# AutoAILab/FusionDepth

Hardware: AMD Instinct MI355X
Metric: training images/sec (640x192, ResNet-18, 4-beam) (higher is better)
Workload: dtype f32

## Files before the change

fusiondepth_amd/csrc/conv.hip:

```cpp
#include "../../include/fdhip.h"
#include "fd_common.h"
#include "conv_fast.h"
#include "conv_generic.h"
#include "conv_wino.h"
#include "conv_limb.h"
#include <stdio.h>
#include <algorithm>
#include "conv_narrow.h"

extern "C" int fd_axpby(const float* a, const float* b, float* out, long n, float alpha, float beta, void* stream);
extern "C" int fd_act_bwd(const float* y, const float* gy, float* gpre, long n, int act, void* stream);

namespace {

__global__ void k_reduce_slabs(const float* __restrict__ slabs, float* __restrict__ out, long n, int splits, int accumulate) {
    for (long i = (long)blockIdx.x * blockDim.x + threadIdx.x; i < n; i += (long)gridDim.x * blockDim.x) {
        float s = accumulate ? out[i] : 0.f;
        for (int z = 0; z < splits; ++z) s += slabs[(long)z * n + i];
        out[i] = s;
    }
}

__global__ void k_weight_relayout(const float* __restrict__ W, float* __restrict__ Wt, int Co, int Ci, int KH, int KW,
                                  int TA, int TB, int kh0, int dkh, int kw0, int dkw) {
// ... 633 lines not shown
        FD_REQUIRE(gy && w && gx, "fd_conv2d_bwd_data: NULL tensor");
        if (int rc = c1_dgrad_launch(d, gy, w, gx, st)) return rc;
        return add_after();
    }
    FD_REQUIRE(gy && w && gx && wt_base, "fd_conv2d_bwd_data: NULL tensor");
    ConvShape s;
    FD_REQUIRE(conv_out_shape(d, s), "fd_conv2d_bwd_data: empty output");
    FD_REQUIRE((long)d->N * d->Cin * (d->H + 2) * (d->W + 2) < (1L << 29) && (long)d->N * d->Cout * s.Ho * s.Wo < (1L << 29),
               "fd_conv2d_bwd_data: tensor too large for 32-bit byte offsets (2 GiB per tensor)");
    const int KH = d->KH, KW = d->KW;
    const long pad_n = d->pad_mode == 1 ? align4((long)d->N * d->Cin * (d->H + 2) * (d->W + 2)) : 0;
    FD_REQUIRE(ws || (pad_n == 0), "fd_conv2d_bwd_data: workspace required for reflect padding");
    float* gpad = ws;
    float* slabs = ws ? ws + pad_n : nullptr;
    if (!wt_ready && d->stride == 1)
        if (int rc = relayout_launch(r, d, w, wt_base, st)) return rc;

    switch (r.fam) {
    case Fam::LIMB_1X1:
        return limb_gemm_launch(wt_base, gy, gx, nullptr, gx_add, ws, d->Cin, d->Cout, d->N, d->H * d->W, 0, st);
    case Fam::WINO:
        return wino_conv_launch(&r.g, gy, wt_base, nullptr, gx, ws, st, gx_add);
    case Fam::WINO_PADDED: {
        const long planes_in = (long)d->N * d->Cout, bx = ((long)(d->H + 2) * (d->W + 2) + 255) / 256;
        float* gyp = slabs + wino_ws_floats(&r.g);
        hipLaunchKernelGGL(k_zero_border_copy, dim3((unsigned)(bx > 64 ? 64 : bx), (unsigned)(planes_in > 32768 ? 32768 : planes_in)), dim3(256), 0, st,
                           gy, gyp, planes_in, d->H, d->W);
        FD_LAUNCH_CHECK("fd_conv2d_bwd_data(zero border)");
        if (int rc = wino_conv_launch(&r.g, gyp, wt_base, nullptr, gpad, slabs, st, nullptr)) return rc;
        reflect_fold_launch(gpad, gx, d, st);
        FD_LAUNCH_CHECK("fd_conv2d_bwd_data(fold)");
        return add_after();
    }
    default: break;
    }
    const bool fast = r.fam != Fam::GENERIC;

    GemmProblem g = {};
    g.X = gy; g.bias = nullptr; g.act = 0; g.in_norm = 0; g.pad_mode = 0;
    g.M = d->Cin; g.Nb = d->N; g.C = d->Cout; g.Hi = s.Ho; g.Wi = s.Wo;
    auto run = [&](const float* A, int TA, int TB, const float* add) -> int {
        if (fast) {
            FastGemmArgs f = {};
            f.A = A; f.X = gy; f.Y = g.Y; f.bias = nullptr;
            f.M = d->Cin; f.C = d->Cout; f.T = TA * TB; f.TB = TB; f.K = f.T * f.C;
            f.Nb = d->N; f.Hi = s.Ho; f.Wi = s.Wo; f.NY = g.NY; f.NX = g.NX;
            f.sy = g.sy; f.oy = g.oy; f.da = g.da; f.sx = g.sx; f.ox = g.ox; f.db = g.db;
            f.pad_mode = 0;
            f.out_ns = g.out_ns; f.out_cs = g.out_cs; f.out_w = g.out_w;
            f.osy = g.osy; f.ooy = g.ooy; f.osx = g.osx; f.oox = g.oox;
            f.out_total = (long)d->N * g.out_ns; f.slab_stride = f.out_total;
            f.slabs = slabs;
            f.add = add;
            return fast_gemm_launch(f, st);
        }
        g.A = A; g.K = d->Cout * TA * TB;
        if (int rc = dispatch_gemm(TA, TB, g, st)) return rc;
        FD_LAUNCH_CHECK("fd_conv2d_bwd_data(gemm)");
        return 0;
    };

    if (d->stride == 1) {
        g.sy = 1; g.da = 1; g.sx = 1; g.db = 1;
        g.osy = 1; g.ooy = 0; g.osx = 1; g.oox = 0;
        if (r.fam == Fam::RING_WINO || r.fam == Fam::RING_N16 || r.fam == Fam::RING_DIRECT) {
            g.NY = d->H; g.NX = d->W; g.oy = -1; g.ox = -1;
            g.Y = gx; g.out_w = d->W; g.out_cs = (long)d->H * d->W; g.out_ns = g.out_cs * d->Cin;
            if (r.fam == Fam::RING_WINO) {
                if (int rc = wino_conv_launch(&r.g, gy, wt_base + r.job[1].off, nullptr, gx, slabs, st, nullptr)) return rc;
            } else if (r.fam == Fam::RING_N16) {
                if (int rc = n16_launch(d, d->Cin, d->Cout, gy, w, nullptr, gx, 1, 0, 0, st)) return rc;
            } else if (int rc = run(wt_base, KH, KW, nullptr)) return rc;
            const int Hp = d->H, Wp2 = d->W + 2;
            const long ring_plane = 2L * Wp2 + 2L * Hp;
            float* ring = gpad;
            FastGemmArgs f = {};
            FastGemmGroup q = {};
            f.A = wt_base; f.X = gy; f.Y = ring; f.bias = nullptr;
            f.M = d->Cin; f.C = d->Cout; f.T = 9; f.TB = 3; f.K = 9 * d->Cout;
            f.Nb = d->N; f.Hi = s.Ho; f.Wi = s.Wo;
            f.sy = 1; f.da = 1; f.sx = 1; f.db = 1; f.pad_mode = 0;
            f.osy = 1; f.osx = 1; f.ooy = 0; f.oox = 0;
            f.out_total = (long)d->N * d->Cin * ring_plane; f.slab_stride = f.out_total; f.slabs = nullptr; f.add = nullptr;
            q.n = 4; q.own_out = 1;
            const int ny[4] = {1, 1, Hp, Hp}, nx[4] = {Wp2, Wp2, 1, 1};
            const int oy4[4] = {-2, -2 + d->H + 1, -1, -1}, ox4[4] = {-2, -2, -2, -2 + d->W + 1};
            const long yoff[4] = {0, Wp2, 2L * Wp2, 2L * Wp2 + Hp};
            for (int j = 0; j < 4; ++j) {
                q.A[j] = wt_base; q.NY[j] = ny[j]; q.NX[j] = nx[j]; q.oy[j] = oy4[j]; q.ox[j] = ox4[j]; q.ooy[j] = 0; q.oox[j] = 0;
                q.T[j] = 9; q.TB[j] = 3; q.K[j] = 9 * d->Cout;
                q.y_off[j] = yoff[j]; q.out_w[j] = nx[j]; q.out_cs[j] = ring_plane; q.out_ns[j] = ring_plane * d->Cin;
            }
            f.NY = q.NY[0]; f.NX = q.NX[0]; f.oy = q.oy[0]; f.ox = q.ox[0];
            f.out_w = q.out_w[0]; f.out_cs = q.out_cs[0]; f.out_ns = q.out_ns[0];
            if (int rc = fast_gemm_group_launch(f, q, st)) return rc;
            const long planes = (long)d->N * d->Cin;
            const int rows2 = (d->H - 2 != 1) ? 2 : 1, cols2 = (d->W - 2 != 1) ? 2 : 1;
            const long targets = planes * ((long)rows2 * d->W + (long)(d->H - rows2) * cols2);
            hipLaunchKernelGGL(k_reflect_ring_fold, dim3((unsigned)ew_blocks(targets)), dim3(256), 0, st, ring, gx, planes, d->H, d->W);
            FD_LAUNCH_CHECK("fd_conv2d_bwd_data(ring fold)");
            return add_after();
        }
        if (d->pad_mode == 1) {
            g.NY = d->H + 2; g.NX = d->W + 2; g.oy = -(KH - 1); g.ox = -(KW - 1);
            g.Y = gpad; g.out_w = d->W + 2;
            g.out_cs = (long)(d->H + 2) * (d->W + 2); g.out_ns = g.out_cs * d->Cin;
            if (int rc = run(wt_base, KH, KW, nullptr)) return rc;
            reflect_fold_launch(gpad, gx, d, st);
            FD_LAUNCH_CHECK("fd_conv2d_bwd_data(fold)");
            return add_after();
        }
        g.NY = d->H; g.NX = d->W; g.oy = -(KH - 1 - d->pad); g.ox = -(KW - 1 - d->pad);
        g.Y = gx; g.out_w = d->W; g.out_cs = (long)d->H * d->W; g.out_ns = g.out_cs * d->Cin;
        const float* add = fast ? gx_add : nullptr;
        if (int rc = run(wt_base, KH, KW, add)) return rc;
        return add ? 0 : add_after();
    }
    g.out_w = d->W; g.out_cs = (long)d->H * d->W; g.out_ns = g.out_cs * d->Cin; g.Y = gx;
    FD_REQUIRE(!r.need_zero || hipMemsetAsync(gx, 0, sizeof(float) * (size_t)gx_n, st) == hipSuccess, "fd_conv2d_bwd_data: memset failed");
    const float* add = fast && !r.need_zero ? gx_add : nullptr;
    if (fast) {
        FastGemmArgs f = {};
        FastGemmGroup q = {};
        f.X = gy; f.Y = gx; f.bias = nullptr;
        f.M = d->Cin; f.C = d->Cout;
        f.Nb = d->N; f.Hi = s.Ho; f.Wi = s.Wo;
        f.sy = 1; f.da = -1; f.sx = 1; f.db = -1;
        f.pad_mode = 0;
        f.out_ns = g.out_ns; f.out_cs = g.out_cs; f.out_w = g.out_w;
        f.osy = 2; f.osx = 2;
        f.out_total = (long)d->N * g.out_ns; f.slab_stride = f.out_total; f.slabs = nullptr;
        f.add = add;
        for (int i = r.njobs - 1; i >= 0; --i) {
            const Job& c = r.job[i];
            if (!wt_ready)
                if (int rc = relayout_launch(r, d, w, wt_base, st, i, 1)) return rc;
            const int j = q.n++;
            q.A[j] = wt_base + c.off; q.NY[j] = (d->H - c.ph + 1) / 2; q.NX[j] = (d->W - c.pw + 1) / 2;
            q.oy[j] = (c.ph + d->pad - c.kh0) / 2; q.ox[j] = (c.pw + d->pad - c.kw0) / 2;
            q.ooy[j] = c.ph; q.oox[j] = c.pw;
            q.T[j] = c.TA * c.TB; q.TB[j] = c.TB; q.K[j] = c.TA * c.TB * d->Cout;
        }
        if (q.n > 0) {
            f.A = q.A[0]; f.NY = q.NY[0]; f.NX = q.NX[0]; f.T = q.T[0]; f.TB = q.TB[0]; f.K = q.K[0];
            if (r.fam == Fam::LIMB_S2) { if (int rc = limb_conv_group_launch(f, q, st)) return rc; }
            else if (int rc = fast_gemm_group_launch(f, q, st)) return rc;
        }
        return add ? 0 : add_after();
    }
    for (int i = 0; i < r.njobs; ++i) {
        const Job& c = r.job[i];
        if (!wt_ready)
            if (int rc = relayout_launch(r, d, w, wt_base, st, i, 1)) return rc;
        g.NY = (d->H - c.ph + 1) / 2; g.NX = (d->W - c.pw + 1) / 2;
        g.sy = 1; g.oy = (c.ph + d->pad - c.kh0) / 2; g.da = -1;
        g.sx = 1; g.ox = (c.pw + d->pad - c.kw0) / 2; g.db = -1;
        g.osy = 2; g.ooy = c.ph; g.osx = 2; g.oox = c.pw;
        if (int rc = run(wt_base + c.off, c.TA, c.TB, nullptr)) return rc;
    }
    return add_after();
}
}

extern "C" long fd_conv2d_fwd_wt_floats(const fd_conv_desc* d) { return d ? route_fwd(d).wt : 0; }
extern "C" long fd_conv2d_fwd_ws_floats(const fd_conv_desc* d) { return d ? route_fwd(d).ws : 0; }

extern "C" int fd_conv2d_fwd(const fd_conv_desc* d, const float* x, const float* w, const float* bias, float* y, float* wt,
                             int wt_ready, float* ws, void* stream) {
    if (int rc = check_desc(d, "fd_conv2d_fwd")) return rc;
    return conv2d_fwd_impl(d, route_fwd(d), x, w, bias, y, wt, wt_ready, ws, nullptr, (hipStream_t)stream);
}
extern "C" int fd_conv2d_fwd_bn_ok(const fd_conv_desc* d, int groups) {
    if (!d || check_desc(d, "fd_conv2d_fwd_bn_ok")) return 0;
    return route_fwd(d).bn && bn_small_slabs_ok(d->N, d->Cout, d->H, d->W, groups) ? 1 : 0;
}
extern "C" int fd_conv2d_fwd_bn(const fd_conv_desc* d, const float* x, const float* w, float* y, float* wt, int wt_ready, float* ws,
                                const float* bn_weight, const float* bn_bias, const float* residual, float* out, float* running_mean,
// ... 151 lines not shown
```

fusiondepth_amd/csrc/conv_fast.h:

```cpp
#pragma once
#include <hip/hip_runtime.h>
#include "../../include/fdhip.h"

struct FastGemmArgs {
    const float* A;
    const float* X;
    float* Y;
    const float* bias;
    float* slabs;
    long slab_stride, out_total;
    int M, K;
    int Nb, C, Hi, Wi;
    int NY, NX;
    int T, TB;
    int sy, oy, da, sx, ox, db;
    int pad_mode;
    long out_ns, out_cs;
    int out_w, osy, ooy, osx, oox;
    int act;
    int xcd_swizzle;
    const float* add;
};

struct FastGemmGroup {
    const float* A[4];
    int NY[4], NX[4], oy[4], ox[4], ooy[4], oox[4], T[4], TB[4], K[4];
    long y_off[4], out_ns[4], out_cs[4];
    int out_w[4];
    int own_out;
    int first_bx[5];
    int n;
};

struct FastWgradArgs {
    const float* dY; const float* X; float* slabs;
    int M, C, T, TB;
    int Nb, Hi, Wi, NY, NX;
    int sy, oy, da, sx, ox, db;
    int pad_mode;
    long dy_ns, dy_cs;
    long pix_per_split;
};

long fast_splitk_slab_floats(const FastGemmArgs& a, int* splits_out);
int fast_gemm_launch(const FastGemmArgs& a, hipStream_t st);
int fast_gemm_group_launch(const FastGemmArgs& a, const FastGemmGroup& q, hipStream_t st);
int fast_weight_relayout(const float* W, float* A2, int Co, int Ci, int KH, int KW, int TA, int TB, int kh0, int dkh, int kw0,
                         int dkw, int mode, hipStream_t st);
int fast_wgrad_splits(int M, int C, int T, long Np);
int fast_wgrad_launch(const FastWgradArgs& a, float* gw, int splits, int accumulate, hipStream_t st);

int fast_splitk_finish_launch(const float* slabs, float* Y, const float* bias, long total, long slab_stride, int splits, long out_cs,
                              int M, int act, hipStream_t st, const float* add = nullptr);

bool n16_shape_ok(const fd_conv_desc* d, int M, int C);
int n16_launch(const fd_conv_desc* d, int M, int C, const float* x, const float* w, const float* bias, float* y, int flip,
               int pad_mode, int act, hipStream_t st);
bool c1_shape_ok(const fd_conv_desc* d);
int c1_fwd_launch(const fd_conv_desc* d, const float* x, const float* w, const float* bias, float* y, hipStream_t st);
int c1_dgrad_launch(const fd_conv_desc* d, const float* gy, const float* w, float* gx, hipStream_t st, const float* x_in = nullptr, int in_act = 0);
bool stem7_fwd_ok(const fd_conv_desc* d);
int stem7_fwd_launch(const fd_conv_desc* d, const float* x, const float* w, const float* bias, float* y, hipStream_t st);
int fast_wgrad_finish_launch(const float* slabs, float* gw, int M, int C, int T, int splits, int accumulate, hipStream_t st);

bool limb_fwd_ok(const fd_conv_desc* d);
bool limb_dgrad_ok(const fd_conv_desc* d);
bool limb_wgrad_ok(const fd_conv_desc* d);
long limb_wt_floats(long M, long K);
long limb_gemm_ws_floats(int M, int K, int Nb, int HW);
int limb_weight_split_launch(const float* w, float* wt, int M, int K, int transposed, hipStream_t st);
int limb_gemm_launch(const float* wt, const float* x, float* y, const float* bias, const float* add, float* ws, int M, int K, int Nb, int HW,
                     int act, hipStream_t st);
long limb_wgrad_ws_floats(int M, int C, int Nb, int HW);
int limb_wgrad_launch(const float* x, const float* gy, float* gw, float* ws, int M, int C, int Nb, int HW, int accumulate, hipStream_t st);
bool limb_conv_problem_ok(int M, int C, int pad_mode, int act);
int limb_conv_weight_split_launch(const float* w, float* wt, int Co, int Ci, int KH, int KW, int TA, int TB, int kh0, int dkh, int kw0, int dkw,
                                  int mode, hipStream_t st);
long limb_conv_ws_floats(const FastGemmArgs& a);
int limb_conv_launch(const FastGemmArgs& a, hipStream_t st);
int limb_conv_group_launch(const FastGemmArgs& a, const FastGemmGroup& q, hipStream_t st);
bool limb_wgrad_s2_shape_ok(int M, int C, int Hi, int Wi, int NY, int NX);
long limb_wgrad_s2_ws_floats(int M, int C, int Nb, int plane, int ntaps);
int limb_wgrad_s2_launch(const float* x, const float* gy, float* gw, float* ws, int M, int C, int Nb, int Hi, int Wi, int NY, int NX, int ntaps,
                         int accumulate, hipStream_t st);
bool limb_conv_1x1_worth(int M, long Np);
```

fusiondepth_amd/csrc/conv_fast.hip:

```cpp
#include "../../include/fdhip.h"
#include "fd_common.h"
#include "conv_fast.h"
#include <type_traits>
#include <stdlib.h>
#include <stdio.h>

#ifndef FD_LS_DIV
#define FD_LS_DIV 2
#endif
namespace {

typedef float f32x16 __attribute__((ext_vector_type(16)));

__device__ __attribute__((noinline)) float act_apply_slow(float v, int act) {
    if (act == 2) return v > 0.f ? v : expm1f(v);
    if (act == 3) return 1.0f / (1.0f + expf(-v));
    return tanhf(v);
}
__device__ __forceinline__ float act_apply(float v, int act) {
    if (act >= 2) return act_apply_slow(v, act);
    return act == 1 ? (v > 0.f ? v : 0.f) : v;
}
__device__ __forceinline__ int refl_idx(int i, int n) {
    i = i < 0 ? -i : i;
    return i >= n ? 2 * n - 2 - i : i;
}

template <int WAVES_M, int WAVES_N, int WM, int WN, int BKC>
__device__ __forceinline__ void conv_fast_body(const FastGemmArgs& g, int bx, int ntx) {
    constexpr int NT = 64 * WAVES_M * WAVES_N;
    constexpr int BM = WAVES_M * 32 * WM, BN = WAVES_N * 32 * WN;
    constexpr int LDA = BM + 1, LDB = BN;
    constexpr int RP = NT / BN;
    constexpr int NB_LOAD = BKC / RP;
    constexpr int A_V4_PER_ROW = BKC / 4;
    constexpr int A_ROWS_PER_PASS = NT / A_V4_PER_ROW;
    constexpr int NA_LOAD = (BM + A_ROWS_PER_PASS - 1) / A_ROWS_PER_PASS;
    constexpr bool A_PARTIAL = (BM % A_ROWS_PER_PASS) != 0;
    static_assert(NT % BN == 0 && BKC % RP == 0, "tile/loader mismatch");
    extern __shared__ __attribute__((aligned(16))) float smem[];
    float* sA = smem;
    float* sB = smem + 2 * BKC * LDA;

    const int tid = threadIdx.x, lane = tid & 63, wave = tid >> 6;
    const int wave_m = wave / WAVES_N, wave_n = wave % WAVES_N;
    if (g.xcd_swizzle) { const int per = ntx >> 3; bx = (bx & 7) * per + (bx >> 3); }
    const int m0 = blockIdx.y * BM;
    const long p0 = (long)bx * BN;
    const int plane = g.NY * g.NX;
    const long Np = (long)g.Nb * plane;
    const unsigned chw = (unsigned)(g.Hi * g.Wi);
    const int cpt = g.C / BKC;
    const int nchunk_all = g.T * cpt;
    const int nsplit = (int)gridDim.z, zs = (int)blockIdx.z;
    const int per_split = (nchunk_all + nsplit - 1) / nsplit;
    const int ch_lo = zs * per_split;
    const int ch_hi = ch_lo + per_split < nchunk_all ? ch_lo + per_split : nchunk_all;

    const int jn = tid % BN;
    const int kr = __builtin_amdgcn_readfirstlane(tid / BN);
    const long pg = p0 + jn;
    const bool pvalid = pg < Np;
    int ry0, cx0;
    unsigned nbase;
    {
        const long pp = pvalid ? pg : 0;
        const int n = (int)(pp / plane);
        const int rem = (int)(pp - (long)n * plane);
        const int y = rem / g.NX, x = rem - y * g.NX;
        ry0 = y * g.sy + g.oy; cx0 = x * g.sx + g.ox;
        nbase = (unsigned)n * (unsigned)g.C * chw;
    }
    const int a4 = tid % A_V4_PER_ROW, ar = tid / A_V4_PER_ROW;

    const __amdgpu_buffer_rsrc_t rsA = fd_make_rsrc(g.A), rsX = fd_make_rsrc(g.X);
    float4 ra[NA_LOAD];
    float rb[NB_LOAD];
    unsigned a_off[NA_LOAD], b_off = FD_OOB;
    const unsigned b_step = 4u * (unsigned)RP * chw;
    int pc_ta, pc_tb, pc_c0;
    { const int t = ch_lo / cpt; pc_c0 = (ch_lo - t * cpt) * BKC; pc_ta = t / g.TB; pc_tb = t - pc_ta * g.TB; }
    const bool refl = g.pad_mode == 1;
    auto prep_chunk = [&](bool live) __attribute__((always_inline)) {
        const unsigned k0 = (unsigned)(pc_ta * g.TB + pc_tb) * (unsigned)g.C + (unsigned)pc_c0;
#pragma unroll
        for (int i = 0; i < NA_LOAD; ++i) {
            int m = m0 + ar + A_ROWS_PER_PASS * i;
            m = m < g.M ? m : g.M - 1;
            a_off[i] = live ? 4u * ((unsigned)m * (unsigned)g.K + k0 + 4u * a4) : FD_OOB;
        }
        int r = ry0 + pc_ta * g.da, cc = cx0 + pc_tb * g.db;
        const bool inb = ((unsigned)r < (unsigned)g.Hi) & ((unsigned)cc < (unsigned)g.Wi);
        const int rr = refl_idx(r, g.Hi), rc = refl_idx(cc, g.Wi);
        r = refl ? rr : r; cc = refl ? rc : cc;
        const bool ok = pvalid & live & (refl | inb);
        b_off = ok ? 4u * (nbase + (unsigned)(pc_c0 + kr) * chw + (unsigned)(r * g.Wi + cc)) : FD_OOB;
        pc_c0 += BKC;
        if (pc_c0 >= g.C) { pc_c0 = 0; ++pc_tb; if (pc_tb >= g.TB) { pc_tb = 0; ++pc_ta; } }
    };
    auto load_a = [&](int i) __attribute__((always_inline)) {
        if (!A_PARTIAL || ar + A_ROWS_PER_PASS * i < BM) ra[i] = fd_ldg128(rsA, a_off[i]);
    };
    auto load_b = [&](int i) __attribute__((always_inline)) { rb[i] = fd_ldg32(rsX, b_off + (unsigned)i * b_step); };
    auto store_a = [&](int buf, int i) __attribute__((always_inline)) {
        if (A_PARTIAL && ar + A_ROWS_PER_PASS * i >= BM) return;
        float* q = sA + buf * BKC * LDA + (4 * a4) * LDA + ar + A_ROWS_PER_PASS * i;
        q[0] = ra[i].x; q[LDA] = ra[i].y; q[2 * LDA] = ra[i].z; q[3 * LDA] = ra[i].w;
    };
    auto store_b = [&](int buf, int i) __attribute__((always_inline)) {
        sB[buf * BKC * LDB + (kr + RP * i) * LDB + jn] = rb[i];
    };

    f32x16 acc[WM][WN];
#pragma unroll
    for (int i = 0; i < WM; ++i)
#pragma unroll
        for (int j = 0; j < WN; ++j)
#pragma unroll
            for (int r = 0; r < 16; ++r) acc[i][j][r] = 0.f;

    constexpr int NK = BKC / 2;
    constexpr int LS = NK / FD_LS_DIV;
    const int arow = lane >> 5, acol = lane & 31;
    if (ch_lo < ch_hi) {
        prep_chunk(true);
#pragma unroll
        for (int i = 0; i < NA_LOAD; ++i) load_a(i);
#pragma unroll
        for (int i = 0; i < NB_LOAD; ++i) load_b(i);
#pragma unroll
        for (int i = 0; i < NA_LOAD; ++i) store_a(0, i);
#pragma unroll
        for (int i = 0; i < NB_LOAD; ++i) store_b(0, i);
        __syncthreads();
        for (int ch = ch_lo; ch < ch_hi; ++ch) {
            const int cur = (ch - ch_lo) & 1;
            prep_chunk(ch + 1 < ch_hi);
            const float* pa = sA + cur * BKC * LDA + arow * LDA + wave_m * 32 * WM + acol;
            const float* pb = sB + cur * BKC * LDB + arow * LDB + wave_n * 32 * WN + acol;
            float av[2][WM], bv[2][WN];
#pragma unroll
            for (int i = 0; i < WM; ++i) av[0][i] = pa[i * 32];
#pragma unroll
            for (int j = 0; j < WN; ++j) bv[0][j] = pb[j * 32];
#pragma unroll
            for (int kk = 0; kk < NK; ++kk) {
                const int cb = kk & 1, nb = cb ^ 1;
                if (kk + 1 < NK) {
#pragma unroll
                    for (int i = 0; i < WM; ++i) av[nb][i] = pa[(kk + 1) * 2 * LDA + i * 32];
#pragma unroll
                    for (int j = 0; j < WN; ++j) bv[nb][j] = pb[(kk + 1) * 2 * LDB + j * 32];
                }
                if (kk < LS) {
#pragma unroll
                    for (int i = 0; i < NA_LOAD; ++i) if ((i * LS) / NA_LOAD == kk) load_a(i);
#pragma unroll
                    for (int i = 0; i < NB_LOAD; ++i) if ((i * LS) / NB_LOAD == kk) load_b(i);
                } else if (kk >= NK - LS) {
#pragma unroll
                    for (int i = 0; i < NA_LOAD; ++i) if ((i * LS) / NA_LOAD == kk - (NK - LS)) store_a(cur ^ 1, i);
#pragma unroll
                    for (int i = 0; i < NB_LOAD; ++i) if ((i * LS) / NB_LOAD == kk - (NK - LS)) store_b(cur ^ 1, i);
                }
                __builtin_amdgcn_sched_barrier(0);
#pragma unroll
                for (int i = 0; i < WM; ++i)
#pragma unroll
                    for (int j = 0; j < WN; ++j)
                        acc[i][j] = __builtin_amdgcn_mfma_f32_32x32x2f32(av[cb][i], bv[cb][j], acc[i][j], 0, 0, 0);
                __builtin_amdgcn_sched_barrier(0);
            }
            __syncthreads();
        }
    }

    const bool final_pass = nsplit == 1;
    const __amdgpu_buffer_rsrc_t rsY = fd_make_rsrc(final_pass ? g.Y : g.slabs + (size_t)blockIdx.z * g.slab_stride);
    const __amdgpu_buffer_rsrc_t rsAdd = fd_make_rsrc(g.add ? g.add : g.Y);
    const bool has_add = final_pass && g.add;
    const unsigned cs4 = 4u * (unsigned)g.out_cs;
    float bias_r[WM][16];
#pragma unroll
    for (int i = 0; i < WM; ++i)
#pragma unroll
        for (int r = 0; r < 16; ++r) bias_r[i][r] = 0.f;
    if (final_pass && g.bias) {
#pragma unroll
        for (int i = 0; i < WM; ++i)
#pragma unroll
            for (int r = 0; r < 16; ++r) {
                const int m = m0 + wave_m * 32 * WM + i * 32 + (r & 3) + 8 * (r >> 2) + 4 * arow;
                bias_r[i][r] = g.bias[m < g.M ? m : g.M - 1];
            }
    }
    auto rows = [&](auto act_tag) __attribute__((always_inline)) {
        constexpr int ACT = decltype(act_tag)::value;
#pragma unroll
        for (int j = 0; j < WN; ++j) {
            const long p = p0 + wave_n * 32 * WN + j * 32 + acol;
            unsigned pix = FD_OOB;
            if (p < Np) {
                const int n = (int)(p / plane);
                const int rem = (int)(p - (long)n * plane);
                const int y = rem / g.NX, x = rem - y * g.NX;
                pix = 4u * (unsigned)((long)n * g.out_ns + (long)(y * g.osy + g.ooy) * g.out_w + (x * g.osx + g.oox));
            }
            unsigned off[WM][16];
            float addv[WM][16];
#pragma unroll
            for (int i = 0; i < WM; ++i)
#pragma unroll
                for (int r = 0; r < 16; ++r) {
                    const int m = m0 + wave_m * 32 * WM + i * 32 + (r & 3) + 8 * (r >> 2) + 4 * arow;
                    off[i][r] = (m < g.M) ? pix + (unsigned)m * cs4 : FD_OOB;
                    addv[i][r] = 0.f;
                }
            if (has_add) {
#pragma unroll
                for (int i = 0; i < WM; ++i)
#pragma unroll
                    for (int r = 0; r < 16; ++r) addv[i][r] = fd_ldg32(rsAdd, off[i][r]);
            }
#pragma unroll
            for (int i = 0; i < WM; ++i)
#pragma unroll
                for (int r = 0; r < 16; ++r) {
                    float v = acc[i][j][r];
                    if (final_pass) {
                        v += bias_r[i][r];
                        if (ACT != 0) v = act_apply(v, g.act);
                        v += addv[i][r];
                    }
                    __builtin_amdgcn_raw_buffer_store_b32(__builtin_bit_cast(unsigned, v), rsY, (int)off[i][r], 0, 0);
                }
        }
    };
    if (g.act == 0 || !final_pass) rows(std::integral_constant<int, 0>{});
    else rows(std::integral_constant<int, -1>{});
}

template <int WAVES_M, int WAVES_N, int WM, int WN, int BKC>
__global__ void __launch_bounds__(64 * WAVES_M * WAVES_N) k_conv_fast(FastGemmArgs g) {
    conv_fast_body<WAVES_M, WAVES_N, WM, WN, BKC>(g, (int)blockIdx.x, (int)gridDim.x);
}

template <int WAVES_M, int WAVES_N, int WM, int WN, int BKC>
__global__ void __launch_bounds__(64 * WAVES_M * WAVES_N) k_conv_fast_grp(FastGemmArgs g, FastGemmGroup q) {
    int j = 0;
    while (j + 1 < q.n && (int)blockIdx.x >= q.first_bx[j + 1]) ++j;
    g.A = q.A[j]; g.NY = q.NY[j]; g.NX = q.NX[j]; g.oy = q.oy[j]; g.ox = q.ox[j]; g.ooy = q.ooy[j]; g.oox = q.oox[j];
    g.T = q.T[j]; g.TB = q.TB[j]; g.K = q.K[j];
    if (q.own_out) { g.Y += q.y_off[j]; g.out_ns = q.out_ns[j]; g.out_cs = q.out_cs[j]; g.out_w = q.out_w[j]; }
    g.xcd_swizzle = 0;
    conv_fast_body<WAVES_M, WAVES_N, WM, WN, BKC>(g, (int)blockIdx.x - q.first_bx[j], q.first_bx[j + 1] - q.first_bx[j]);
}

__global__ void __launch_bounds__(256) k_splitk_finish(const float* __restrict__ slabs, float* __restrict__ Y,
                                                       const float* __restrict__ bias, long total, long slab_stride,
                                                       int splits, long out_cs, int M, int act, const float* __restrict__ add) {
    const unsigned cs = (unsigned)out_cs, uM = (unsigned)M;
    for (unsigned i = blockIdx.x * 256u + threadIdx.x; i < (unsigned)total; i += gridDim.x * 256u) {
        float s = 0.f;
        int z = 0;
        for (; z + 4 <= splits; z += 4) {
            const float a0 = slabs[(size_t)z * slab_stride + i], a1 = slabs[(size_t)(z + 1) * slab_stride + i];
            const float a2 = slabs[(size_t)(z + 2) * slab_stride + i], a3 = slabs[(size_t)(z + 3) * slab_stride + i];
            s += a0; s += a1; s += a2; s += a3;
        }
        for (; z < splits; ++z) s += slabs[(size_t)z * slab_stride + i];
        if (bias) s += bias[(i / cs) % uM];
        s = act_apply(s, act);
        if (add) s += add[i];
        Y[i] = s;
    }
}

template <int WAVES_M, int WAVES_N, int WM, int WN>
__global__ void __launch_bounds__(64 * WAVES_M * WAVES_N) k_wgrad_fast(FastWgradArgs g) {
    constexpr int NT = 64 * WAVES_M * WAVES_N;
    constexpr int BM = WAVES_M * 32 * WM, BN = WAVES_N * 32 * WN;
    constexpr int BP = 32;
    constexpr int LDA = BM + 1, LDB = BN + 1;
    constexpr int RPW = NT / BP;
    constexpr int NA_LOAD = BM / RPW, NB_LOAD = BN / RPW;
    extern __shared__ __attribute__((aligned(16))) float smem[];
    float* sA = smem;
    float* sB = smem + 2 * BP * LDA;

    const int tid = threadIdx.x, lane = tid & 63, wave = tid >> 6;
    const int wave_m = wave / WAVES_N, wave_n = wave % WAVES_N;
    const int cblocks = (g.C + BN - 1) / BN;
    const int t = blockIdx.x / cblocks, c0 = (blockIdx.x - t * cblocks) * BN;
    const int ta = t / g.TB, tb = t - ta * g.TB;
    const int m0 = blockIdx.y * BM;
    const int plane = g.NY * g.NX;
    const long Np = (long)g.Nb * plane;
    const unsigned chw = (unsigned)(g.Hi * g.Wi);
    const long pbeg = (long)blockIdx.z * g.pix_per_split;
    long pend = pbeg + g.pix_per_split;
    if (pend > Np) pend = Np;

    const int pl = tid % BP, rw = tid / BP;
    const int ncol = g.C - c0 < BN ? g.C - c0 : BN;
    const int nrow = g.M - m0 < BM ? g.M - m0 : BM;

    const __amdgpu_buffer_rsrc_t rsY = fd_make_rsrc(g.dY), rsX = fd_make_rsrc(g.X);
    float ra[NA_LOAD], rb[NB_LOAD];
    unsigned rowa[NA_LOAD], rowb[NB_LOAD];
#pragma unroll
    for (int i = 0; i < NA_LOAD; ++i) {
        const int r = rw + RPW * i < nrow ? rw + RPW * i : nrow - 1;
        rowa[i] = 4u * (unsigned)(m0 + r) * (unsigned)g.dy_cs;
    }
#pragma unroll
    for (int i = 0; i < NB_LOAD; ++i) {
        const int c = rw + RPW * i < ncol ? rw + RPW * i : ncol - 1;
        rowb[i] = 4u * (unsigned)(c0 + c) * chw;
    }
    unsigned offa = FD_OOB, offb = FD_OOB;
    int pn, prem;
    { const long p = pbeg + pl; pn = (int)(p / plane); prem = (int)(p - (long)pn * plane); }
    long pcur = pbeg + pl;
    const float inv_nx = 1.0f / (float)g.NX;
    const bool refl = g.pad_mode == 1;
    auto prep_chunk = [&]() __attribute__((always_inline)) {
        const bool pv = pcur < pend;
        int y = (int)(((float)prem + 0.5f) * inv_nx);
        int x = prem - y * g.NX;
        if (x < 0) { --y; x += g.NX; }
        if (x >= g.NX) { ++y; x -= g.NX; }
        offa = pv ? 4u * ((unsigned)pn * (unsigned)g.dy_ns + (unsigned)prem) : FD_OOB;
        int r = y * g.sy + g.oy + ta * g.da, cc = x * g.sx + g.ox + tb * g.db;
        const bool inb = ((unsigned)r < (unsigned)g.Hi) & ((unsigned)cc < (unsigned)g.Wi);
        const int rr = refl_idx(r, g.Hi), rc = refl_idx(cc, g.Wi);
        r = refl ? rr : r; cc = refl ? rc : cc;
        const bool ok = pv & (refl | inb);
        offb = ok ? 4u * ((unsigned)pn * (unsigned)g.C * chw + (unsigned)(r * g.Wi + cc)) : FD_OOB;
// ... 157 lines not shown
                const float h = 0.5f * (t1 + t2);
                v = ky == 0 ? t0 + h : (ky == 1 ? 0.5f * (t1 - t2) : h - t3);
            }
            o[i * os] = old[i] + v;
        }
    }
}

__global__ void __launch_bounds__(256) k_weight_relayout_tc(const float* __restrict__ W, float* __restrict__ A2, int Co,
                                                            int Ci, int KH, int KW, int TA, int TB, int kh0, int dkh, int kw0,
                                                            int dkw, int mode) {
    const int Mr = mode ? Ci : Co, Cr = mode ? Co : Ci;
    const long n = (long)Mr * TA * TB * Cr;
    for (long i = (long)blockIdx.x * 256 + threadIdx.x; i < n; i += (long)gridDim.x * 256) {
        const int c = (int)(i % Cr);
        const int b = (int)((i / Cr) % TB);
        const int a = (int)((i / ((long)Cr * TB)) % TA);
        const int m = (int)(i / ((long)Cr * TB * TA));
        const int co = mode ? c : m, ci = mode ? m : c;
        A2[i] = W[(((long)co * Ci + ci) * KH + kh0 + dkh * a) * KW + kw0 + dkw * b];
    }
}

inline int ew_blocks(long n) {
    long b = (n + 255) / 256;
    return (int)(b < 1 ? 1 : (b > 4096 ? 4096 : b));
}

template <int WAVES_M, int WAVES_N, int WM, int WN, int BKC>
void launch_cfg(const FastGemmArgs& a, int splits, hipStream_t st) {
    constexpr int BM = WAVES_M * 32 * WM, BN = WAVES_N * 32 * WN;
    const long Np = (long)a.Nb * a.NY * a.NX;
    const int gx = fd_cdiv(Np, BN), gy = fd_cdiv(a.M, BM);
    FastGemmArgs g = a;
    g.xcd_swizzle = (gx % 8 == 0 && gx >= 16) ? 1 : 0;
    const size_t lds = sizeof(float) * 2 * BKC * ((BM + 1) + BN);
    fd_launch_lds<k_conv_fast<WAVES_M, WAVES_N, WM, WN, BKC>>(dim3(gx, gy, splits), dim3(64 * WAVES_M * WAVES_N), lds, st, g);
}

}

namespace {
struct FastChoice { int cfg; int splits; };
FastChoice choose_config(const FastGemmArgs& a) {
    if (fd_tun().force_cfg >= 0) {
        const int c = fd_tun().force_cfg, sp = fd_tun().force_splits;
        const bool ok_c = (c == 0 && a.M > 64) || (c == 1 && a.M > 32) || c == 2;
        const bool can = a.osy == 1 && a.osx == 1 && a.slab_stride > 0;
        if (ok_c) return {c, can ? sp : 1};
    }
    const long Np = (long)a.Nb * a.NY * a.NX;
    const int bkc = (a.C % 32 == 0) ? 32 : 16;
    const int nchunk = a.T * (a.C / bkc);
    const bool can_split = a.osy == 1 && a.osx == 1 && a.slab_stride > 0;
    const int bm[3] = {128, 64, 32}, bn[3] = {128, 128, 256};
    const int c = a.M > 32 ? 1 : 2;
    const long tiles = (long)fd_cdiv(Np, bn[c]) * fd_cdiv(a.M, bm[c]);
    const long fill = fd_tun().conv_target;
    int sp = 1;
    if (can_split && tiles < fill) {
        sp = (int)(fill / tiles);
        const int cap = nchunk / 4 > 0 ? (nchunk / 4 < 16 ? nchunk / 4 : 16) : 1;
        if (sp > cap) sp = cap;
        if (sp < 1) sp = 1;
    }
    return {c, sp};
}
}

long fast_splitk_slab_floats(const FastGemmArgs& a, int* splits_out) {
    FastGemmArgs probe = a;
    if (probe.slab_stride <= 0) probe.slab_stride = probe.out_total > 0 ? probe.out_total : 1;
    const FastChoice ch = choose_config(probe);
    if (splits_out) *splits_out = ch.splits;
    return ch.splits > 1 ? (long)ch.splits * a.out_total : 0;
}

namespace {
template <int WAVES_M, int WAVES_N, int WM, int WN, int BKC>
void launch_grp(const FastGemmArgs& a, const FastGemmGroup& q, hipStream_t st) {
    constexpr int BM = WAVES_M * 32 * WM, BN = WAVES_N * 32 * WN;
    FastGemmGroup grp = q;
    int gx = 0;
    for (int j = 0; j < q.n; ++j) { grp.first_bx[j] = gx; gx += fd_cdiv((long)a.Nb * q.NY[j] * q.NX[j], BN); }
    grp.first_bx[q.n] = gx;
    const size_t lds = sizeof(float) * 2 * BKC * ((BM + 1) + BN);
    fd_launch_lds<k_conv_fast_grp<WAVES_M, WAVES_N, WM, WN, BKC>>(dim3(gx, fd_cdiv(a.M, BM), 1), dim3(64 * WAVES_M * WAVES_N), lds, st, a, grp);
}
}

int fast_gemm_group_launch(const FastGemmArgs& a, const FastGemmGroup& q, hipStream_t st) {
    if ((double)a.Nb * a.C * a.Hi * a.Wi * 4.0 >= 2147483648.0) { fd_set_error("conv: tensor exceeds the 2 GiB addressing range of the fast path"); return -1; }
    for (int j = 0; j < q.n; ++j)
        if ((double)a.M * q.K[j] * 4.0 >= 2147483648.0) { fd_set_error("conv: weights exceed the 2 GiB addressing range of the fast path"); return -1; }
    const bool b32 = a.C % 32 == 0;
    long wgs128 = 0;
    for (int j = 0; j < q.n; ++j) wgs128 += fd_cdiv((long)a.Nb * q.NY[j] * q.NX[j], 128) * fd_cdiv(a.M, 64);
    if (a.M > 32 && b32 && wgs128 < (long)fd_tun().grp_tile64_below) launch_grp<2, 2, 1, 1, 32>(a, q, st);
    else if (a.M > 32) { if (b32) launch_grp<2, 2, 1, 2, 32>(a, q, st); else launch_grp<2, 2, 1, 2, 16>(a, q, st); }
    else { if (b32) launch_grp<1, 4, 1, 2, 32>(a, q, st); else launch_grp<1, 4, 1, 2, 16>(a, q, st); }
    hipError_t e = hipGetLastError();
    if (e != hipSuccess) { fd_set_error("k_conv_fast_grp launch failed: %s", hipGetErrorString(e)); return (int)e; }
    return 0;
}

int fast_gemm_launch(const FastGemmArgs& a, hipStream_t st) {
    if ((double)a.Nb * a.C * a.Hi * a.Wi * 4.0 >= 2147483648.0 || (double)a.M * a.K * 4.0 >= 2147483648.0) {
        fd_set_error("conv: tensor exceeds the 2 GiB addressing range of the fast path"); return -1;
    }
    const FastChoice ch = choose_config(a);
    const int splits = ch.splits;
    if (splits > 1 && !a.slabs) { fd_set_error("conv: split-K workspace missing"); return -1; }
    const bool b32 = a.C % 32 == 0;
    if (ch.cfg == 0) {
        if (b32) launch_cfg<2, 2, 2, 2, 32>(a, splits, st); else launch_cfg<2, 2, 2, 2, 16>(a, splits, st);
    } else if (ch.cfg == 1) {
        if (b32) launch_cfg<2, 2, 1, 2, 32>(a, splits, st); else launch_cfg<2, 2, 1, 2, 16>(a, splits, st);
    } else {
        if (b32) launch_cfg<1, 4, 1, 2, 32>(a, splits, st); else launch_cfg<1, 4, 1, 2, 16>(a, splits, st);
    }
    hipError_t e = hipGetLastError();
    if (e != hipSuccess) { fd_set_error("k_conv_fast launch failed: %s", hipGetErrorString(e)); return (int)e; }
    if (splits > 1)
        return fast_splitk_finish_launch(a.slabs, a.Y, a.bias, a.out_total, a.slab_stride, splits, a.out_cs, a.M, a.act, st, a.add);
    return 0;
}

int fast_wgrad_finish_launch(const float* slabs, float* gw, int M, int C, int T, int splits, int accumulate, hipStream_t st) {
    if ((T == 9 && C % 32 == 0) || T == 12) {
        const int cb = (C + 31) / 32;
        int mb = (int)(((long)M * cb) / 1024);
        mb = mb < 1 ? 1 : (mb > 8 ? 8 : mb);
        const dim3 grid(cb, (M + mb - 1) / mb);
#define FD_FIN9(CH, ZU)                                                                                                    \
    do {                                                                                                                   \
        if (T == 9) hipLaunchKernelGGL((k_wgrad_finish9<9, CH, ZU>), grid, dim3(384), 0, st, slabs, gw, M, C, splits, accumulate, mb); \
        else hipLaunchKernelGGL((k_wgrad_finish9<12, CH, ZU>), grid, dim3(384), 0, st, slabs, gw, M, C, splits, accumulate, mb);       \
    } while (0)
        static_assert(FIN9_MB == 8, "the mb rule above and the CH choice below end at 8 channels");
        if (mb == 1) FD_FIN9(1, 16);
        else if (mb == 2) FD_FIN9(2, 8);
        else if (mb <= 4) FD_FIN9(4, 4);
        else if (splits > 1) FD_FIN9(8, 2);
        else FD_FIN9(8, 1);
#undef FD_FIN9
        hipError_t e9 = hipGetLastError();
        if (e9 != hipSuccess) { fd_set_error("k_wgrad_finish9 launch failed: %s", hipGetErrorString(e9)); return (int)e9; }
        return 0;
    }
    hipLaunchKernelGGL(k_wgrad_finish, dim3(ew_blocks((long)M * C * T)), dim3(256), 0, st, slabs, gw, M, C, T, splits, accumulate);
    hipError_t e = hipGetLastError();
    if (e != hipSuccess) { fd_set_error("k_wgrad_finish launch failed: %s", hipGetErrorString(e)); return (int)e; }
    return 0;
}

int fast_splitk_finish_launch(const float* slabs, float* Y, const float* bias, long total, long slab_stride, int splits, long out_cs,
                              int M, int act, hipStream_t st, const float* add) {
    hipLaunchKernelGGL(k_splitk_finish, dim3(ew_blocks(total)), dim3(256), 0, st, slabs, Y, bias, total, slab_stride, splits, out_cs, M,
                       act, add);
    hipError_t e = hipGetLastError();
    if (e != hipSuccess) { fd_set_error("k_splitk_finish launch failed: %s", hipGetErrorString(e)); return (int)e; }
    return 0;
}

int fast_weight_relayout(const float* W, float* A2, int Co, int Ci, int KH, int KW, int TA, int TB, int kh0, int dkh,
                         int kw0, int dkw, int mode, hipStream_t st) {
    const long n = (long)Co * Ci * TA * TB;
    hipLaunchKernelGGL(k_weight_relayout_tc, dim3(ew_blocks(n)), dim3(256), 0, st, W, A2, Co, Ci, KH, KW, TA, TB, kh0, dkh,
                       kw0, dkw, mode);
    hipError_t e = hipGetLastError();
    if (e != hipSuccess) { fd_set_error("k_weight_relayout_tc launch failed: %s", hipGetErrorString(e)); return (int)e; }
    return 0;
}

int fast_wgrad_splits(int M, int C, int T, long Np) {
    const long target = fd_tun().wgrad_target;
    const int bn = C >= 128 ? 128 : 64;
    const long tiles = (long)T * fd_cdiv(C, bn) * fd_cdiv(M, M > 32 ? 64 : 32);
    long sp = target / tiles;
    const long maxs = (Np + 511) / 512;
    if (sp > maxs) sp = maxs;
// ... 27 lines not shown
```

Measured before the change: 705.7.

## Restrict ring dgrad taps to live window and fold reflection in epilogue

The reflect-pad ring correction in the dgrad path now computes only the kernel taps that actually reach each border strip (a tap window given by ta0/tb0/TBW) instead of all nine. A new ring epilogue accumulates directly into gx, with a fifth group covering the corners, so the separate ring buffer and the reflect-fold kernel are skipped. The small-tile threshold is also raised for these thin groups. This removes redundant MACs, one kernel launch and a round trip through the intermediate buffer. In exchange it adds read-modify-write stores, shuffle-based corner reductions and more complex indexing, which risks correctness bugs and races at overlapping outputs.

```diff
diff --git a/fusiondepth_amd/csrc/conv.hip b/fusiondepth_amd/csrc/conv.hip
--- a/fusiondepth_amd/csrc/conv.hip
+++ b/fusiondepth_amd/csrc/conv.hip
@@ -739,17 +739,31 @@
             f.sy = 1; f.da = 1; f.sx = 1; f.db = 1; f.pad_mode = 0;
             f.osy = 1; f.osx = 1; f.ooy = 0; f.oox = 0;
             f.out_total = (long)d->N * d->Cin * ring_plane; f.slab_stride = f.out_total; f.slabs = nullptr; f.add = nullptr;
-            q.n = 4; q.own_out = 1;
+            q.n = 4; q.own_out = 1; q.thin = 1;
             const int ny[4] = {1, 1, Hp, Hp}, nx[4] = {Wp2, Wp2, 1, 1};
             const int oy4[4] = {-2, -2 + d->H + 1, -1, -1}, ox4[4] = {-2, -2, -2, -2 + d->W + 1};
             const long yoff[4] = {0, Wp2, 2L * Wp2, 2L * Wp2 + Hp};
+            const int ta0[4] = {2, 0, 0, 0}, tb0[4] = {0, 0, 2, 0}, tbn[4] = {3, 3, 1, 1};
             for (int j = 0; j < 4; ++j) {
                 q.A[j] = wt_base; q.NY[j] = ny[j]; q.NX[j] = nx[j]; q.oy[j] = oy4[j]; q.ox[j] = ox4[j]; q.ooy[j] = 0; q.oox[j] = 0;
-                q.T[j] = 9; q.TB[j] = 3; q.K[j] = 9 * d->Cout;
+                q.T[j] = 3; q.TB[j] = tbn[j]; q.K[j] = 9 * d->Cout;
+                q.ta0[j] = ta0[j]; q.tb0[j] = tb0[j]; q.TBW[j] = 3;
                 q.y_off[j] = yoff[j]; q.out_w[j] = nx[j]; q.out_cs[j] = ring_plane; q.out_ns[j] = ring_plane * d->Cin;
             }
             f.NY = q.NY[0]; f.NX = q.NX[0]; f.oy = q.oy[0]; f.ox = q.ox[0];
             f.out_w = q.out_w[0]; f.out_cs = q.out_cs[0]; f.out_ns = q.out_ns[0];
+            if (d->H >= 4 && d->W >= 4) {
+                q.own_out = 0;
+                for (int j = 0; j < 4; ++j) q.ring_kind[j] = j;
+                q.A[4] = wt_base; q.NY[4] = 4; q.NX[4] = 4; q.oy[4] = 0; q.ox[4] = 0; q.ooy[4] = 0; q.oox[4] = 0;
+                q.T[4] = 9; q.TB[4] = 3; q.K[4] = 9 * d->Cout; q.ta0[4] = 0; q.tb0[4] = 0; q.TBW[4] = 3; q.ring_kind[4] = 4;
+                q.n = 5;
+                f.Y = gx; f.ring_h = d->H; f.ring_w = d->W;
+                f.out_w = d->W; f.out_cs = (long)d->H * d->W; f.out_ns = f.out_cs * d->Cin;
+                f.out_total = (long)d->N * f.out_ns; f.slab_stride = f.out_total;
+                if (int rc = fast_gemm_group_launch(f, q, st)) return rc;
+                return add_after();
+            }
             if (int rc = fast_gemm_group_launch(f, q, st)) return rc;
             const long planes = (long)d->N * d->Cin;
             const int rows2 = (d->H - 2 != 1) ? 2 : 1, cols2 = (d->W - 2 != 1) ? 2 : 1;
diff --git a/fusiondepth_amd/csrc/conv_fast.h b/fusiondepth_amd/csrc/conv_fast.h
--- a/fusiondepth_amd/csrc/conv_fast.h
+++ b/fusiondepth_amd/csrc/conv_fast.h
@@ -20,15 +20,23 @@
     int act;
     int xcd_swizzle;
     const float* add;
+    int ta0, tb0, TBW;
+    int ring_h, ring_w;
+    int ring_kind;
 };
 
+constexpr int FAST_GRP_MAX = 5;
 struct FastGemmGroup {
-    const float* A[4];
-    int NY[4], NX[4], oy[4], ox[4], ooy[4], oox[4], T[4], TB[4], K[4];
-    long y_off[4], out_ns[4], out_cs[4];
-    int out_w[4];
+    const float* A[FAST_GRP_MAX];
+    int NY[FAST_GRP_MAX], NX[FAST_GRP_MAX], oy[FAST_GRP_MAX], ox[FAST_GRP_MAX], ooy[FAST_GRP_MAX], oox[FAST_GRP_MAX];
+    int T[FAST_GRP_MAX], TB[FAST_GRP_MAX], K[FAST_GRP_MAX];
+    int ta0[FAST_GRP_MAX], tb0[FAST_GRP_MAX], TBW[FAST_GRP_MAX];
+    int ring_kind[FAST_GRP_MAX];
+    long y_off[FAST_GRP_MAX], out_ns[FAST_GRP_MAX], out_cs[FAST_GRP_MAX];
+    int out_w[FAST_GRP_MAX];
     int own_out;
-    int first_bx[5];
+    int thin;
+    int first_bx[FAST_GRP_MAX + 1];
     int n;
 };
 
diff --git a/fusiondepth_amd/csrc/conv_fast.hip b/fusiondepth_amd/csrc/conv_fast.hip
--- a/fusiondepth_amd/csrc/conv_fast.hip
+++ b/fusiondepth_amd/csrc/conv_fast.hip
@@ -1,6 +1,7 @@
 #include "../../include/fdhip.h"
 #include "fd_common.h"
 #include "conv_fast.h"
+#include <algorithm>
 #include <type_traits>
 #include <stdlib.h>
 #include <stdio.h>
@@ -26,7 +27,8 @@
     return i >= n ? 2 * n - 2 - i : i;
 }
 
-template <int WAVES_M, int WAVES_N, int WM, int WN, int BKC>
+constexpr int EPI_STORE = 0, EPI_RING = 1;
+template <int WAVES_M, int WAVES_N, int WM, int WN, int BKC, bool WIN = false, int EPI = EPI_STORE>
 __device__ __forceinline__ void conv_fast_body(const FastGemmArgs& g, int bx, int ntx) {
     constexpr int NT = 64 * WAVES_M * WAVES_N;
     constexpr int BM = WAVES_M * 32 * WM, BN = WAVES_N * 32 * WN;
@@ -60,7 +62,7 @@
     const int jn = tid % BN;
     const int kr = __builtin_amdgcn_readfirstlane(tid / BN);
     const long pg = p0 + jn;
-    const bool pvalid = pg < Np;
+    bool pvalid = pg < Np;
     int ry0, cx0;
     unsigned nbase;
     {
@@ -70,6 +72,12 @@
         const int y = rem / g.NX, x = rem - y * g.NX;
         ry0 = y * g.sy + g.oy; cx0 = x * g.sx + g.ox;
         nbase = (unsigned)n * (unsigned)g.C * chw;
+        if (EPI == EPI_RING && g.ring_kind == 4) {
+            const int py = x == 2 ? ((y >> 1) ? g.ring_h - 1 : 2) : ((y >> 1) ? g.ring_h + 1 : 0);
+            const int px = x == 0 ? ((y & 1) ? g.ring_w - 1 : 2) : ((y & 1) ? g.ring_w + 1 : 0);
+            ry0 = py - 2; cx0 = px - 2;
+            pvalid = pvalid && x < 3;
+        }
     }
     const int a4 = tid % A_V4_PER_ROW, ar = tid / A_V4_PER_ROW;
 
@@ -79,10 +87,12 @@
     unsigned a_off[NA_LOAD], b_off = FD_OOB;
     const unsigned b_step = 4u * (unsigned)RP * chw;
     int pc_ta, pc_tb, pc_c0;
-    { const int t = ch_lo / cpt; pc_c0 = (ch_lo - t * cpt) * BKC; pc_ta = t / g.TB; pc_tb = t - pc_ta * g.TB; }
+    const int tb_lo = WIN ? g.tb0 : 0, tb_hi = tb_lo + g.TB, tbw = WIN ? g.TBW : g.TB;
+    { const int t = ch_lo / cpt; pc_c0 = (ch_lo - t * cpt) * BKC; pc_ta = t / g.TB; pc_tb = t - pc_ta * g.TB + tb_lo; }
+    if (WIN) pc_ta += g.ta0;
     const bool refl = g.pad_mode == 1;
     auto prep_chunk = [&](bool live) __attribute__((always_inline)) {
-        const unsigned k0 = (unsigned)(pc_ta * g.TB + pc_tb) * (unsigned)g.C + (unsigned)pc_c0;
+        const unsigned k0 = (unsigned)(pc_ta * tbw + pc_tb) * (unsigned)g.C + (unsigned)pc_c0;
 #pragma unroll
         for (int i = 0; i < NA_LOAD; ++i) {
             int m = m0 + ar + A_ROWS_PER_PASS * i;
@@ -96,7 +106,7 @@
         const bool ok = pvalid & live & (refl | inb);
         b_off = ok ? 4u * (nbase + (unsigned)(pc_c0 + kr) * chw + (unsigned)(r * g.Wi + cc)) : FD_OOB;
         pc_c0 += BKC;
-        if (pc_c0 >= g.C) { pc_c0 = 0; ++pc_tb; if (pc_tb >= g.TB) { pc_tb = 0; ++pc_ta; } }
+        if (pc_c0 >= g.C) { pc_c0 = 0; ++pc_tb; if (pc_tb >= tb_hi) { pc_tb = tb_lo; ++pc_ta; } }
     };
     auto load_a = [&](int i) __attribute__((always_inline)) {
         if (!A_PARTIAL || ar + A_ROWS_PER_PASS * i < BM) ra[i] = fd_ldg128(rsA, a_off[i]);
@@ -236,6 +246,45 @@
                 }
         }
     };
+    if constexpr (EPI == EPI_RING) {
+        const int H = g.ring_h, W = g.ring_w, kind = g.ring_kind;
+#pragma unroll
+        for (int j = 0; j < WN; ++j) {
+            const long p = p0 + wave_n * 32 * WN + j * 32 + acol;
+            unsigned pix = FD_OOB;
+            if (p < Np) {
+                const int n = (int)(p / plane);
+                const int rem = (int)(p - (long)n * plane);
+                const int y = rem / g.NX, x = rem - y * g.NX;
+                int ty, tx;
+                bool on;
+                if (kind <= 1) { on = !(x == 0 || x == 2 || x == W - 1 || x == W + 1); ty = kind ? H - 2 : 1; tx = x - 1; }
+                else if (kind <= 3) { on = !(y == 1 || y == H - 2); ty = y; tx = kind == 3 ? W - 2 : 1; }
+                else { on = x == 0; ty = (y >> 1) ? H - 2 : 1; tx = (y & 1) ? W - 2 : 1; }
+                if (on) pix = 4u * (unsigned)((long)n * g.out_ns + (long)ty * W + tx);
+            }
+            unsigned off[WM][16];
+            float old[WM][16];
+#pragma unroll
+            for (int i = 0; i < WM; ++i)
+#pragma unroll
+                for (int r = 0; r < 16; ++r) {
+                    const int m = m0 + wave_m * 32 * WM + i * 32 + (r & 3) + 8 * (r >> 2) + 4 * arow;
+                    off[i][r] = (m < g.M) ? pix + (unsigned)m * cs4 : FD_OOB;
+                    old[i][r] = fd_ldg32(rsY, off[i][r]);
+                }
+#pragma unroll
+            for (int i = 0; i < WM; ++i)
+#pragma unroll
+                for (int r = 0; r < 16; ++r) {
+                    const float v = acc[i][j][r];
+                    float s = 0.f + v;
+                    if (kind == 4) { s += __shfl_down(v, 1); s += __shfl_down(v, 2); }
+                    __builtin_amdgcn_raw_buffer_store_b32(__builtin_bit_cast(unsigned, old[i][r] + s), rsY, (int)off[i][r], 0, 0);
+                }
+        }
+        return;
+    }
     if (g.act == 0 || !final_pass) rows(std::integral_constant<int, 0>{});
     else rows(std::integral_constant<int, -1>{});
 }
@@ -245,15 +294,16 @@
     conv_fast_body<WAVES_M, WAVES_N, WM, WN, BKC>(g, (int)blockIdx.x, (int)gridDim.x);
 }
 
-template <int WAVES_M, int WAVES_N, int WM, int WN, int BKC>
+template <int WAVES_M, int WAVES_N, int WM, int WN, int BKC, int EPI>
 __global__ void __launch_bounds__(64 * WAVES_M * WAVES_N) k_conv_fast_grp(FastGemmArgs g, FastGemmGroup q) {
     int j = 0;
     while (j + 1 < q.n && (int)blockIdx.x >= q.first_bx[j + 1]) ++j;
     g.A = q.A[j]; g.NY = q.NY[j]; g.NX = q.NX[j]; g.oy = q.oy[j]; g.ox = q.ox[j]; g.ooy = q.ooy[j]; g.oox = q.oox[j];
     g.T = q.T[j]; g.TB = q.TB[j]; g.K = q.K[j];
+    g.ta0 = q.ta0[j]; g.tb0 = q.tb0[j]; g.TBW = q.TBW[j]; g.ring_kind = q.ring_kind[j];
     if (q.own_out) { g.Y += q.y_off[j]; g.out_ns = q.out_ns[j]; g.out_cs = q.out_cs[j]; g.out_w = q.out_w[j]; }
     g.xcd_swizzle = 0;
-    conv_fast_body<WAVES_M, WAVES_N, WM, WN, BKC>(g, (int)blockIdx.x - q.first_bx[j], q.first_bx[j + 1] - q.first_bx[j]);
+    conv_fast_body<WAVES_M, WAVES_N, WM, WN, BKC, true, EPI>(g, (int)blockIdx.x - q.first_bx[j], q.first_bx[j + 1] - q.first_bx[j]);
 }
 
 __global__ void __launch_bounds__(256) k_splitk_finish(const float* __restrict__ slabs, float* __restrict__ Y,
@@ -577,10 +627,15 @@
     constexpr int BM = WAVES_M * 32 * WM, BN = WAVES_N * 32 * WN;
     FastGemmGroup grp = q;
     int gx = 0;
-    for (int j = 0; j < q.n; ++j) { grp.first_bx[j] = gx; gx += fd_cdiv((long)a.Nb * q.NY[j] * q.NX[j], BN); }
+    for (int j = 0; j < q.n; ++j) {
+        grp.first_bx[j] = gx; gx += fd_cdiv((long)a.Nb * q.NY[j] * q.NX[j], BN);
+        if (grp.TBW[j] == 0) { grp.TBW[j] = q.TB[j]; grp.ta0[j] = 0; grp.tb0[j] = 0; }
+    }
     grp.first_bx[q.n] = gx;
     const size_t lds = sizeof(float) * 2 * BKC * ((BM + 1) + BN);
-    fd_launch_lds<k_conv_fast_grp<WAVES_M, WAVES_N, WM, WN, BKC>>(dim3(gx, fd_cdiv(a.M, BM), 1), dim3(64 * WAVES_M * WAVES_N), lds, st, a, grp);
+    const dim3 grid(gx, fd_cdiv(a.M, BM), 1), block(64 * WAVES_M * WAVES_N);
+    if (a.ring_h) fd_launch_lds<k_conv_fast_grp<WAVES_M, WAVES_N, WM, WN, BKC, EPI_RING>>(grid, block, lds, st, a, grp);
+    else fd_launch_lds<k_conv_fast_grp<WAVES_M, WAVES_N, WM, WN, BKC, EPI_STORE>>(grid, block, lds, st, a, grp);
 }
 }
 
@@ -591,7 +646,8 @@
     const bool b32 = a.C % 32 == 0;
     long wgs128 = 0;
     for (int j = 0; j < q.n; ++j) wgs128 += fd_cdiv((long)a.Nb * q.NY[j] * q.NX[j], 128) * fd_cdiv(a.M, 64);
-    if (a.M > 32 && b32 && wgs128 < (long)fd_tun().grp_tile64_below) launch_grp<2, 2, 1, 1, 32>(a, q, st);
+    const long tile64_below = q.thin ? std::max(256L, (long)fd_tun().grp_tile64_below) : (long)fd_tun().grp_tile64_below;
+    if (a.M > 32 && b32 && wgs128 < tile64_below) launch_grp<2, 2, 1, 1, 32>(a, q, st);
     else if (a.M > 32) { if (b32) launch_grp<2, 2, 1, 2, 32>(a, q, st); else launch_grp<2, 2, 1, 2, 16>(a, q, st); }
     else { if (b32) launch_grp<1, 4, 1, 2, 32>(a, q, st); else launch_grp<1, 4, 1, 2, 16>(a, q, st); }
     hipError_t e = hipGetLastError();
```

New measurement: 710.2 (median of 6 runs). No clear change (+0.6%).
